# haowenz/chromap

Measured on AMD Instinct MI355X. Metric: M paired reads mapped/s (ATAC preset, GRCh38 index), higher is better.
Workload: dtype u64; 1 GPU; --preset atac, synthetic 2x50 bp pairs (fragments 30-600 bp, 1% substitutions), GRCh38-sized synthetic index (3.10e+09 bases, 24 sequences, k=17 w=7) resident per GPU, 4000000 pairs per GPU per step, 4 distinct batches per GPU resident in HBM taking turns (16 M distinct pairs per GPU); lanes=3, parallelism=single GPU

## Files before the change

chromap_amd/csrc/cm_api.hip:

```cpp
#include <hip/hip_runtime.h>
#include <math.h>
#include <stdio.h>
#include <stdlib.h>
#include <string.h>

#include <string>
#include <vector>

#include "../../include/chromap_amd.h"
#include "cm_barcode_translate.h"
#include "cm_ctx.h"
#include "cm_kernels.h"
#include "cm_classes.h"
#include "cm_summary.h"
#include "cm_coop.h"
#include <chrono>
#include <mutex>
#include "cm_mapq_tables.h"

static thread_local std::string g_last_error;

static bool cm_debug_pool() { static const bool on = getenv("CM_DEBUG_POOL") != nullptr; return on; }
static thread_local std::string t_last_error;
void cm_set_error(cmgpu_ctx *ctx, const std::string &msg) {
// ... 86 lines not shown
    c->opt.sam_group = (int)value;
  } else if (n == "verify_planes") {
    c->opt.planes = value ? 1 : 0;
  } else if (n == "speculative_sizes") {
    c->opt.spec = value ? 1 : 0;
    if (value < 0) { c->cls_seen = 0; memset(c->cls_age, 0, sizeof(c->cls_age)); }
  } else if (n == "debug_candidate_capacity") {
    if (value > 0 && cm_ensure_candidate_arrays(c, (uint64_t)value)) { cm_set_error(c, "out of device memory (candidates)"); return CMGPU_ENOMEM; }
    c->pred_m_ok = value > 0; c->m_cap = (uint64_t)value; c->pred_n = 0xffffffffu;
  } else if (n == "coop_profile") {
    if (value) { if (c->coop_prof.ensure(64 * 8)) return CMGPU_ENOMEM; CM_HIPCHECK(c, hipMemset(c->coop_prof.p, 0, 64 * 8)); } else c->coop_prof.release();
  } else if (n == "coop_run_table") {
    c->opt.coop_rb = (int)value;
  } else if (n == "coop") {
    c->opt.coop = (int)value;
  } else if (n == "s3b_short") {
    c->opt.s3b_short = value ? 1 : 0;
  } else if (n == "generic_kernels") {
    c->opt.generic_kernels = value ? 1 : 0;
  } else if (n == "item_limit") {
    c->opt.item_limit = value > 0 ? (uint64_t)value : 0xfffffff0ull;
  } else {
    cm_set_error(c, "unknown option " + n);
    return CMGPU_EINVAL;
  }
  return CMGPU_OK;
}

extern "C" int cmgpu_get_option(const cmgpu_ctx *c, const char *name, int64_t *value) {
  if (!c || !name || !value) return CMGPU_EINVAL;
  const std::string n(name);
  if (n == "probe_lookups_per_lane") *value = c->opt.probe_variant & 15;
  else if (n == "probe_pair_prefetch") *value = (c->opt.probe_variant & 16) ? 1 : 0;
  else if (n == "mm_chunks") *value = c->opt.mm_chunks;
  else if (n == "h2d_copy_blocks") *value = c->opt.h2d_kernel;
  else if (n == "d2h_copy_blocks") *value = c->opt.d2h_kernel;
  else if (n == "prep_kernel") *value = c->opt.prep_kernel;
  else if (n == "prep_tile_reads") *value = c->opt.prep_tile_reads;
  else if (n == "item_limit") *value = (int64_t)c->opt.item_limit;
  else if (n == "lanes") *value = c->opt.lanes;
  else if (n == "coop") *value = c->opt.coop;
  else if (n == "generic_kernels") *value = c->opt.generic_kernels;
  else if (n == "s3b_short") *value = c->opt.s3b_short;
  else if (n == "alloc_us") *value = (int64_t)(c->alloc_seconds * 1e6);
  else if (n == "alloc_draw_us") *value = (int64_t)(c->alloc_draw_seconds * 1e6);
  else if (n.rfind("coop_profile_", 0) == 0) {
    const int k = atoi(n.c_str() + 13);
    unsigned long long v = 0;
    if (k < 0 || k > 63 || !c->coop_prof.p || hipMemcpy(&v, (const unsigned long long *)c->coop_prof.p + k, 8, hipMemcpyDeviceToHost) != hipSuccess) return CMGPU_EINVAL;
    *value = (int64_t)v;
  }
  else if (n == "probe_table_buckets") *value = c->fmask ? (int64_t)c->fmask + 1 : (int64_t)c->bmask + 1;
  else return CMGPU_EINVAL;
  return CMGPU_OK;
}

extern "C" const char *cmgpu_last_error(const cmgpu_ctx *ctx) { return ctx ? ctx->err.c_str() : g_last_error.c_str(); }

// ... 621 lines not shown
#define CM_RC_AGAIN_ALL_CLASSES (-101)
#define CM_RC_AGAIN_EXACT_SIZES (-102)
struct RangeRun {
  cmgpu_ctx *c;
  uint32_t rlo, rhi, n, n2;
  bool allow_spec;
  uint64_t limit;
  hipStream_t s;
  CmDev d;
  uint32_t n_mm = 0;
  bool s3a_done = false;
  uint32_t n_heavy[CM_HV_LISTS] = {};
  unsigned long long hits_total = 0;
  uint32_t n_hits = 0;
  bool planes = false;
  bool spec = false;
  uint32_t n_m = 0;
  void bind() { cm_bind_dev(c, d, rlo, rhi); }
};
static int stage_begin(RangeRun &r) {
  cmgpu_ctx *c = r.c;
  c->n_ev = 0;
  c->use_perm = false;
  const int rc = ensure_pair_arrays(c, r.n);
  if (rc) return rc;
  CM_HIPCHECK(c, hipMemsetAsync(c->stats.p, 0, CM_ST_N * 8, r.s));
  memset(&r.d, 0, sizeof(r.d));
  cm_ensure_goff(c);
  cm_set_classes(c, r.d);
  r.bind();
// ... 19 lines not shown
static int mm_fill_and_probe(RangeRun &r, const MmChunks &k, uint32_t mm_cap, Fill fill) {
  cmgpu_ctx *c = r.c;
  const unsigned long long *marks = (const unsigned long long *)c->mm_marks.p;
  CM_HIPCHECK(c, hipMemsetAsync(r.d.stats + CM_ST_PROBE_STEPS, 0, 2 * 8, r.s));
  for (uint32_t ch = 0; ch < k.n_chunks; ++ch) {
    fill(ch);
    CM_HIPCHECK(c, hipEventRecord(c->chunk_ev[ch], r.s));
    CM_HIPCHECK(c, hipStreamWaitEvent(c->stream2, c->chunk_ev[ch], 0));
    cm_launch_k_probe_range(r.d, marks + ch, k.entries[ch], mm_cap, (uint2 *)c->partials.p + k.part_off[ch], c->stream2, c->opt.probe_variant);
  }
  CM_HIPCHECK(c, hipEventRecord(c->chunk_ev[CM_MM_CHUNKS], c->stream2));
  CM_HIPCHECK(c, hipStreamWaitEvent(r.s, c->chunk_ev[CM_MM_CHUNKS], 0));
  cm_launch_k_probe_reduce(c->partials.p, k.part_off[k.n_chunks], r.d.stats + CM_ST_PROBE_STEPS, r.s);
  return CMGPU_OK;
}
static int stage_minimizers_fused(RangeRun &r, bool flat) {
  cmgpu_ctx *c = r.c; CmDev &d = r.d; hipStream_t s = r.s;
  const uint32_t n = r.n, n2 = r.n2;
  int rc;
  uint64_t cap = (uint64_t)n2 * (c->max_read_len / 4 + 3);
  const uint64_t bound = (uint64_t)c->bases0 + c->bases1 + 1;
  if (cap > bound) cap = bound;
  const uint32_t ppb = flat ? 128u : cm_prep_mm_pairs_per_block(d, c->max_read_len);
  const uint64_t per_read_bound = c->max_read_len > (uint32_t)c->p.k ? c->max_read_len - (uint32_t)c->p.k + 1 : 1;
  MmChunks k;
  k.n_chunks = mm_chunk_count(r);
  for (int attempt = 0; attempt < 2; ++attempt) {
    if (cap > r.limit) return CM_RC_SPLIT;
    k.lo[0] = 0;
    uint32_t chunk_pairs = 0;
    for (uint32_t ch = 0; ch < k.n_chunks; ++ch) {
      uint64_t hi = (uint64_t)n * (ch + 1) / k.n_chunks;
      hi = ch + 1 == k.n_chunks ? n : hi / ppb * ppb;
      k.lo[ch + 1] = (uint32_t)hi;
// ... 3 lines not shown
      k.entries[ch] = me > cap ? cap : me;
    }
    mm_probe_grids(c, k);
    if (c->mm_hash.ensure((size_t)cap * 8 + 8) || c->mm_ps.ensure((size_t)cap * 4 + 4) || c->pr_val.ensure((size_t)cap * 8 + 8) ||
        (!flat && c->mm_stage.ensure(cm_prep_mm_stage_bytes(d, c->max_read_len, chunk_pairs) + 8)) ||
        c->pr_kind.ensure((size_t)cap + 4) || c->mm_cursor.ensure(8) || c->mm_marks.ensure((CM_MM_CHUNKS + 1) * 8) ||
        c->partials.ensure(((size_t)k.part_off[k.n_chunks] + 1) * 8 + cm_stats_partial_words(n) * 8)) {
      cm_set_error(c, "out of device memory (minimizers)"); return CMGPU_ENOMEM;
    }
    r.bind();
    CM_HIPCHECK(c, hipMemsetAsync(c->mm_cursor.p, 0, 8, s));
    CM_HIPCHECK(c, hipMemsetAsync(c->mm_marks.p, 0, 8, s));
    unsigned long long *cursor = (unsigned long long *)c->mm_cursor.p, *marks = (unsigned long long *)c->mm_marks.p;
    rc = mm_fill_and_probe(r, k, (uint32_t)cap, [&](uint32_t ch) {
      if (flat) cm_launch_k_prep_flat(d, k.lo[ch], k.lo[ch + 1], c->max_read_len, (uint32_t)c->opt.prep_tile_reads, (uint32_t)cap, cursor, s);
      else cm_launch_k_prep_mm(d, k.lo[ch], k.lo[ch + 1], c->max_read_len, (uint32_t)cap, cursor, s, c->mm_stage.p);
      cm_launch_k_copy_u64(cursor, marks + ch + 1, s);
    });
    if (rc) return rc;
    d.mm_cap = (uint32_t)cap;
    CM_HIPCHECK(c, hipMemsetAsync(c->hv_cnt.p, 0, 256, s));
    cm_launch_k_s3a_count(d, n2, s);
    d.mm_cap = 0;
    if ((rc = scan_with_total(c, d.hit_tot, d.hit_off, n2, &r.hits_total, false))) return rc;
    CM_HIPCHECK(c, hipMemcpyAsync(r.n_heavy, c->hv_cnt.p, sizeof(r.n_heavy), hipMemcpyDeviceToHost, s));
    r.s3a_done = true;
    unsigned long long hm[CM_MM_CHUNKS + 1];
    CM_HIPCHECK(c, hipMemcpyAsync(hm, marks, ((size_t)k.n_chunks + 1) * 8, hipMemcpyDeviceToHost, s));
    CM_HIPCHECK(c, cm_stream_sync(s));
    const unsigned long long tot = hm[k.n_chunks];
    bool grid_short = false;
// ... 24 lines not shown
  if (c->mm_marks.ensure((CM_MM_CHUNKS + 1) * 8)) { cm_set_error(c, "out of device memory (minimizers)"); return CMGPU_ENOMEM; }
  unsigned long long *marks = (unsigned long long *)c->mm_marks.p;
  unsigned long long hm[CM_MM_CHUNKS + 1];
  cm_launch_k_mm_marks(d.mm_off, k.lo, k.n_chunks + 1, marks, s);
  CM_HIPCHECK(c, hipMemcpyAsync(hm, marks, ((size_t)k.n_chunks + 1) * 8, hipMemcpyDeviceToHost, s));
  CM_HIPCHECK(c, cm_stream_sync(s));
  for (uint32_t ch = 0; ch < k.n_chunks; ++ch) k.entries[ch] = hm[ch + 1] - hm[ch];
  mm_probe_grids(c, k);
  if (c->partials.ensure(((size_t)k.part_off[k.n_chunks] + 1) * 8 + cm_stats_partial_words(r.n) * 8)) { cm_set_error(c, "out of device memory (partials)"); return CMGPU_ENOMEM; }
  if ((rc = mm_fill_and_probe(r, k, n_mm, [&](uint32_t ch) { cm_launch_k_mm_fill(d, k.lo[ch], k.lo[ch + 1], c->max_read_len, s); }))) return rc;
  mark(c, "s1b_s2_minimizers_probe");
  return CMGPU_OK;
}
static int stage_pack_reads(RangeRun &r) {
  cmgpu_ctx *c = r.c;
  r.planes = c->ref_pl_words != 0 && c->opt.planes;
  if (r.planes && c->read_planes.ensure((size_t)r.n2 * cm_read_pl_stride((c->max_read_len + 31) / 32) * 4 + 16)) r.planes = false;
  if (!r.planes) return CMGPU_OK;
  if (!c->stream_pack) {
    int prio_least = 0, prio_greatest = 0;
    (void)hipDeviceGetStreamPriorityRange(&prio_least, &prio_greatest);
    CM_HIPCHECK(c, hipStreamCreateWithPriority(&c->stream_pack, hipStreamNonBlocking, prio_greatest));
  }
  CM_HIPCHECK(c, hipEventRecord(c->chunk_ev[1], r.s));
  CM_HIPCHECK(c, hipStreamWaitEvent(c->stream_pack, c->chunk_ev[1], 0));
  r.d.read_pl = (uint32_t *)c->read_planes.p; r.d.read_pl_w = (c->max_read_len + 31) / 32;
  cm_launch_k_pack_reads(r.d, r.n2, c->stream_pack);
  CM_HIPCHECK(c, hipEventRecord(c->chunk_ev[0], c->stream_pack));
  return CMGPU_OK;
}
static int stage_s3_candidates(RangeRun &r) {
  cmgpu_ctx *c = r.c; CmDev &d = r.d; hipStream_t s = r.s;
// ... 70 lines not shown
  if (cm_debug_pool()) fprintf(stderr, "spec %d m_cap %llu m_total %llu\n", (int)r.spec, (unsigned long long)c->m_cap, m_total);
  r.bind();
  mark(c, "s4a_rescue_count");
  cm_launch_k_s4b_rescue_merge(d, n2, s, coop, c->max_read_len);
  cm_launch_k_s4b_rescue_list(d, n2, s, coop, c->max_read_len);
  mark(c, "s4b_rescue_merge");
  CM_HIPCHECK(c, hipMemsetAsync(c->srt_cnt.p, 0, 8, s));
  cm_launch_k_s4c_reduce(d, r.n, s, (uint32_t)c->opt.coop & (c->p.split ? ~8u : ~0u));
  if (c->use_perm) cm_launch_k_sort_lists(d, 0, s);
  mark(c, "s4c_pair_filter");
  return CMGPU_OK;
}
static int stage_s5_verify(RangeRun &r) {
  cmgpu_ctx *c = r.c; const CmDev &d = r.d; hipStream_t s = r.s;
  const bool coop = (c->opt.coop & 8) != 0 && !c->p.split;
  if (r.planes) CM_HIPCHECK(c, hipStreamWaitEvent(s, c->chunk_ev[0], 0));
  cm_launch_k_s5a_prepare(d, r.n2, s, coop);
  cm_scan_u32(d.nv, d.v_off, r.n2, (uint32_t *)c->scan_tmp.p, s);
  mark(c, "s5a_prepare");
  cm_launch_k_s5b_verify(d, r.n_m, r.n2, s);
  mark(c, "s5b_verify");
  CM_HIPCHECK(c, hipMemsetAsync(c->srt_cnt.p, 0, 8, s));
  cm_launch_k_s5c_finalize(d, r.n2, s, coop);
  if (c->use_perm) cm_launch_k_sort_lists(d, 1, s);
  mark(c, "s5c_accept");
  return CMGPU_OK;
}
static int stage_s6_records(RangeRun &r) {
  cmgpu_ctx *c = r.c; CmDev &d = r.d; hipStream_t s = r.s;
  const uint32_t n = r.n;
  const bool coop = (c->opt.coop & 16) != 0;
// ... 372 lines not shown
    t.force_mapq = c->p.split ? -1 : (f0[i] ? 0 : -1);
  }
  return CMGPU_OK;
}

extern "C" int cmgpu_debug_array(cmgpu_ctx *c, const char *name, uint32_t *out, uint64_t capacity, uint64_t *n_out) {
  if (!c || !name || !out) return CMGPU_EINVAL;
  CM_HIPCHECK(c, cm_enter(c));
  const std::string nm(name);
  if (nm == "hv_cnt") {
    if (n_out) *n_out = 64;
    if (capacity < 64 || !c->hv_cnt.p || c->hv_cnt.cap < 256) { cm_set_error(c, "debug array: buffer too small or array not resident"); return CMGPU_ECAPACITY; }
    CM_HIPCHECK(c, hipMemcpy(out, c->hv_cnt.p, 256, hipMemcpyDeviceToHost));
    return CMGPU_OK;
  }
  struct { const char *n; DevBuf *b; int per_pair; } tab[] = {
    {"rlen", &c->rlen, 0}, {"mm_cnt", &c->mm_cnt, 0}, {"hit_tot", &c->hit_tot, 0}, {"ncp", &c->ncp, 0}, {"ncn", &c->ncn, 0},
    {"resc_p", &c->resc_p, 0}, {"resc_n", &c->resc_n, 0}, {"mcp", &c->mcp, 0}, {"mcn", &c->mcn, 0}, {"fcp", &c->fcp, 0},
    {"fcn", &c->fcn, 0}, {"ndp", &c->ndp, 0}, {"ndn", &c->ndn, 0}, {"nv", &c->nv, 0}, {"pe_nbest", &c->pe_nbest, 1}};
  for (auto &t : tab)
    if (nm == t.n) {
      const uint64_t n = t.per_pair ? c->n_pairs : 2ull * c->n_pairs;
      if (n_out) *n_out = n;
      if (capacity < n || !t.b->p || t.b->cap < n * 4) { cm_set_error(c, "debug array: buffer too small or array not resident"); return CMGPU_ECAPACITY; }
      CM_HIPCHECK(c, hipMemcpy(out, t.b->p, n * 4, hipMemcpyDeviceToHost));
      return CMGPU_OK;
    }
  cm_set_error(c, "debug array: unknown name " + nm);
  return CMGPU_EINVAL;
}
// ... 528 lines not shown
```

chromap_amd/csrc/cm_ctx.h:

```cpp
#ifndef CM_CTX_H_
#define CM_CTX_H_
#include <hip/hip_runtime.h>

#include <string>
#include <thread>
#include <vector>

#include "../../include/chromap_amd.h"
#include "../../include/chromap_amd_debug.h"
#include "cm_types.h"

#define CM_MAX_EVENTS 32
#define CM_MAX_W_HOST 32

struct DevBuf {
  void *p = nullptr;
  size_t cap = 0;
  bool owned = true;
  int ensure(size_t bytes);
  void release();
};

struct CmTmpBuf : private DevBuf {
  using DevBuf::p;
// ... 85 lines not shown
  int sam_group = 8;
  int d2h_kernel = 0;
  int h2d_kernel = 0;
  int probe_variant = 1;
  int mm_chunks = CM_MM_CHUNKS;
  int prep_tile_reads = 32;
  int prep_kernel = 0;
  uint64_t item_limit = 0xfffffff0ull;
  int exchange_overlap = 0;
  int s3b_cap = 0;
  int lanes = 1;
  int heavy_mid = 0;
  int heavy_max[3] = {0, 0, 0};
  int heavy_last = 0;
  int spec = 1;
  int s3b_short = 1;
  int generic_kernels = 0;
  int coop_rb = 0;
  int coop = 0xff;
};

struct cmgpu_ctx {
  CmOptions opt;
  int device = 0;
  hipStream_t stream = nullptr;
  hipStream_t stream2 = nullptr;
  hipStream_t stream_pack = nullptr;
  hipEvent_t chunk_ev[CM_MM_CHUNKS + 1] = {};
  std::string err;
  cmgpu_params hp;
// ... 177 lines not shown
```

chromap_amd/csrc/cm_kernels.h:

```cpp
#ifndef CM_KERNELS_H_
#define CM_KERNELS_H_
#include <hip/hip_runtime.h>

#include "cm_types.h"

#define CM_SLAB_CAP 65535u
#define CM_SLAB_BLOCKS 128u
#define CM_DECL_LAUNCH(kname) void cm_launch_##kname(const CmDev &d, uint32_t n, hipStream_t s);
void cm_launch_k_prep_count(const CmDev &d, uint32_t n_pairs, uint32_t max_read_len, hipStream_t s);
void cm_launch_k_mm_fill(const CmDev &d, uint32_t pair_lo, uint32_t pair_hi, uint32_t max_read_len, hipStream_t s);
void cm_launch_k_mm_marks(const uint32_t *mm_off, const uint32_t *lo, uint32_t n_marks, unsigned long long *marks, hipStream_t s);
bool cm_prep_mm_supported(const CmDev &d, uint32_t max_read_len);
bool cm_prep_flat_supported(const CmDev &d, uint32_t max_read_len, uint32_t tile_reads);
void cm_launch_k_prep_flat(const CmDev &d, uint32_t pair_lo, uint32_t pair_hi, uint32_t max_read_len, uint32_t tile_reads, uint32_t mm_cap,
                           unsigned long long *cursor, hipStream_t s);
uint32_t cm_prep_mm_pairs_per_block(const CmDev &d, uint32_t max_read_len);
size_t cm_prep_mm_stage_bytes(const CmDev &d, uint32_t max_read_len, uint32_t pairs);
void cm_launch_k_prep_mm(const CmDev &d, uint32_t pair_lo, uint32_t pair_hi, uint32_t max_read_len, uint32_t mm_cap,
                         unsigned long long *cursor, hipStream_t s, void *gstage);
uint32_t cm_probe_range_blocks(uint64_t max_entries, int variant);
void cm_launch_k_probe_range(const CmDev &d, const unsigned long long *range, uint64_t max_entries, uint32_t cap, void *partials, hipStream_t s, int variant);
void cm_launch_k_probe_reduce(const void *partials, uint32_t blocks, unsigned long long *counters, hipStream_t s);
CM_DECL_LAUNCH(k_s3a_count)
void cm_launch_k_sort_lists(const CmDev &d, int mode, hipStream_t s);
uint32_t cm_s3b_lane_cap(uint32_t max_read_len);
void cm_s3b_heavy_classes(uint32_t *hv_max, uint32_t *hv_big);
void cm_granted_classes(CmDev &d);
void cm_launch_k_s3b_heavy(const CmDev &d, const uint32_t *n_cls, hipStream_t s, bool coop, uint32_t max_read_len);
void cm_launch_k_s3b_candidates(const CmDev &d, uint32_t n, uint32_t max_read_len, hipStream_t s);
void cm_launch_k_s4a_rescue_count(const CmDev &d, uint32_t n, hipStream_t s, bool coop);
void cm_launch_k_s4b_rescue_merge(const CmDev &d, uint32_t n, hipStream_t s, bool coop, uint32_t max_read_len);
uint32_t cm_rescue_seg_cap(uint32_t n_reads);
void cm_launch_k_s4a_rescue_list(const CmDev &d, uint32_t n_reads, hipStream_t s, bool coop);
void cm_launch_k_s4b_rescue_list(const CmDev &d, uint32_t n_reads, hipStream_t s, bool coop, uint32_t max_read_len);
// ... 30 lines not shown
```

chromap_amd/csrc/cm_kernels.hip:

```cpp
#include <hip/hip_runtime.h>
#include <stdio.h>
#include <string.h>
#include <cstring>
#include <atomic>
#include <map>
#include <mutex>
#include <type_traits>
#include <utility>
#include <rocprim/rocprim.hpp>

#include "cm_kernels.h"
#include "cm_stages.h"
#include "cm_classes.h"
#include "cm_coop.h"

#define CM_BLOCK 256

#define CM_ITEM_KERNEL(kname, fn, perm)                                      \
  __global__ __launch_bounds__(CM_BLOCK) void kname(CmDev d, uint32_t n) {   \
    if (d.abort && *d.abort) return;                                         \
    const uint32_t i = blockIdx.x * CM_BLOCK + threadIdx.x;                  \
    if (i < n) fn(d, d.perm ? d.perm[i] : i);                                \
  }

// ... 27 lines not shown
  const uint32_t t = threadIdx.x, lp = t < PB ? t : t - PB, pair = p0 + lp;
  const CmStaged s = cm_stage_pairs(d, p0, p1, pair, lds_half);
  if (t < PB && pair < p1) cm_s0_prep_ptr(d, pair, s.m0, s.m1);
  __syncthreads();
  if (pair < p1) cm_s1_count(d, 2 * pair + (t < PB ? 0 : 1), t < PB ? s.m0 : s.m1);
}

__global__ void k_mm_fill(CmDev d, uint32_t pair_lo, uint32_t n_pairs , uint32_t lds_half) {
  const uint32_t PB = blockDim.x >> 1;
  const uint32_t p0 = pair_lo + blockIdx.x * PB, p1 = p0 + PB < n_pairs ? p0 + PB : n_pairs;
  const uint32_t t = threadIdx.x, lp = t < PB ? t : t - PB, pair = p0 + lp;
  const CmStaged s = cm_stage_pairs(d, p0, p1, pair, lds_half);
  if (pair < p1) cm_s1_fill(d, 2 * pair + (t < PB ? 0 : 1), t < PB ? s.m0 : s.m1);
}

template <bool GSTAGE, bool E6>
__global__ void k_prep_mm(CmDev d, uint32_t pair_lo, uint32_t n_pairs , uint32_t lds_half, uint32_t stg,
                          uint32_t mm_cap, unsigned long long *cursor, uint64_t *gstage) {
  const uint32_t T = blockDim.x, PB = T >> 1;
  const uint32_t p0 = pair_lo + blockIdx.x * PB, p1 = p0 + PB < n_pairs ? p0 + PB : n_pairs;
  const uint32_t t = threadIdx.x, lp = t < PB ? t : t - PB, pair = p0 + lp;
  const CmStaged s = cm_stage_pairs(d, p0, p1, pair, lds_half);
  if (t < PB && pair < p1) cm_s0_prep_ptr(d, pair, s.m0, s.m1);
  __syncthreads();
  uint64_t *sh_e = GSTAGE ? gstage + (size_t)blockIdx.x * stg * T : reinterpret_cast<uint64_t *>(cm_lds + 2 * lds_half);
  uint32_t *sh_lo = reinterpret_cast<uint32_t *>(cm_lds + 2 * lds_half);
  uint16_t *sh_hi = reinterpret_cast<uint16_t *>(sh_lo + (size_t)stg * T);
  uint32_t *sh_w = reinterpret_cast<uint32_t *>(cm_lds + 2 * lds_half + (GSTAGE ? 0 : (size_t)stg * T * (E6 ? 6 : 8)));
  uint32_t *sh_off = sh_w + 16, *sh_cnt = sh_off + T + 1;
  const bool valid = pair < p1;
  const uint32_t r = 2 * pair + (t < PB ? 0 : 1);
  const uint8_t *seq = t < PB ? s.m0 : s.m1;
  const int k = d.p.k;
  const uint32_t hb = 2 * (uint32_t)k;
  uint32_t cnt = 0, len = 0;
  if (valid) {
    len = d.rlen[r];
    cnt = cm_minimizers_w7(seq, len, k, [&](uint32_t n, uint64_t h, uint32_t p) {
      const uint64_t v = h | ((uint64_t)p << hb);
      if (n < stg) { if (E6) { sh_lo[(size_t)n * T + t] = (uint32_t)v; sh_hi[(size_t)n * T + t] = (uint16_t)(v >> 32); } else sh_e[(size_t)n * T + t] = v; }
    });
  }
  const uint32_t lane = t & 63, wave = t >> 6;
  uint32_t incl = cnt;
#pragma unroll
  for (int dlt = 1; dlt < 64; dlt <<= 1) {
    const uint32_t v = __shfl_up(incl, dlt, 64);
    if (lane >= (uint32_t)dlt) incl += v;
  }
  if (lane == 63 || t == T - 1) sh_w[wave] = incl;
  __syncthreads();
  const uint32_t n_waves = (T + 63) >> 6;
  if (t == 0) {
    uint32_t tot = 0;
    for (uint32_t wv = 0; wv < n_waves; ++wv) { const uint32_t x = sh_w[wv]; sh_w[wv] = tot; tot += x; }
    const unsigned long long base = tot ? atomicAdd(cursor, (unsigned long long)tot) : 0ull;
// ... 1767 lines not shown
  return prep_mm_geometry(d, max_read_len, &t, &h, &g, &l);
}
uint32_t cm_prep_mm_pairs_per_block(const CmDev &d, uint32_t max_read_len) {
  uint32_t threads, half, stg;
  size_t lds;
  return prep_mm_geometry(d, max_read_len, &threads, &half, &stg, &lds) ? threads / 2 : 0;
}
size_t cm_prep_mm_stage_bytes(const CmDev &d, uint32_t max_read_len, uint32_t pairs) {
  uint32_t threads, half, stg;
  size_t lds;
  bool g = false;
  if (!prep_mm_geometry(d, max_read_len, &threads, &half, &stg, &lds, &g) || !g) return 0;
  const uint32_t pb = threads / 2;
  return (size_t)((pairs + pb - 1) / pb) * stg * threads * 8;
}
void cm_launch_k_prep_mm(const CmDev &d, uint32_t pair_lo, uint32_t pair_hi, uint32_t max_read_len, uint32_t mm_cap,
                         unsigned long long *cursor, hipStream_t s, void *gstage) {
  uint32_t threads, half, stg;
  size_t lds;
  bool g = false, e6 = false;
  if (pair_hi <= pair_lo || !prep_mm_geometry(d, max_read_len, &threads, &half, &stg, &lds, &g, &e6)) return;
  const uint32_t pb = threads / 2;
  if (g) hipLaunchKernelGGL((k_prep_mm<true, false>), dim3((pair_hi - pair_lo + pb - 1) / pb), dim3(threads), lds, s, d, pair_lo, pair_hi, half, stg, mm_cap, cursor, (uint64_t *)gstage);
  else if (e6) hipLaunchKernelGGL((k_prep_mm<false, true>), dim3((pair_hi - pair_lo + pb - 1) / pb), dim3(threads), lds, s, d, pair_lo, pair_hi, half, stg, mm_cap, cursor, (uint64_t *)nullptr);
  else hipLaunchKernelGGL((k_prep_mm<false, false>), dim3((pair_hi - pair_lo + pb - 1) / pb), dim3(threads), lds, s, d, pair_lo, pair_hi, half, stg, mm_cap, cursor, (uint64_t *)nullptr);
}
static inline int probe_variant_norm(int variant) {
  if (variant == 0) variant = CM_PROBE_U;
  const int u = variant & 15;
  return ((u == 2 || u == 4 || u == 8) ? u : 1) | (variant & 16);
}
uint32_t cm_probe_range_blocks(uint64_t max_entries, int variant) {
  const uint64_t per = (uint64_t)(probe_variant_norm(variant) & 15) * CM_BLOCK;
  return (uint32_t)((max_entries + per - 1) / per);
}
void cm_launch_k_probe_range(const CmDev &d, const unsigned long long *range, uint64_t max_entries, uint32_t cap, void *partials, hipStream_t s, int variant) {
  const uint32_t blocks = cm_probe_range_blocks(max_entries, variant);
  if (!blocks) return;
// ... 72 lines not shown
```

chromap_amd/csrc/cm_stages.h:

```cpp
#ifndef CM_STAGES_H_
#define CM_STAGES_H_

#include "cm_types.h"

struct CmModeAny {
  static constexpr bool kPe = false;
  static CM_HD bool split(const CmDev &d) { return d.p.split != 0; }
  static CM_HD bool single(const CmDev &d) { return d.p.single != 0; }
};
struct CmModePe {
  static constexpr bool kPe = true;
  static CM_HD bool split(const CmDev &) { return false; }
  static CM_HD bool single(const CmDev &) { return false; }
};

CM_HD uint32_t cm_c2u(uint8_t c) {
  const uint32_t u = c & 0xDFu;
  const uint32_t x = (u >> 1) & 3u;
  const uint32_t o = u - 0x41u;
  const bool acgt = o < 20u && ((0x80045u >> (o & 31u)) & 1u);
  return acgt ? x ^ (x >> 1) : 4u;
}
CM_HD uint8_t cm_negchar(uint8_t c) {
  const uint32_t v = 3u ^ cm_c2u(c);
// ... 400 lines not shown
    }
    const uint64_t r0 = d0 & seedmask;
    const uint64_t r1 = seed >= 32 ? d1 : (((d0 >> (2 * seed)) | (d1 << (64 - 2 * seed))) & seedmask);
    const bool ok = cnt <= 1;
    if (ok && r0 == 0) { fa = true; sa = s0; }
    if (ok && r1 == 0 && !fb) { fb = true; sb = s0; }
#pragma unroll
    for (int w = 0; w + 1 < W; ++w) b[w] = (b[w] >> 2) | (b[w + 1] << 62);
    b[W - 1] >>= 2;
  }
  *found = fa || fb;
  *s0_out = fa ? sa : sb;
  return true;
}

CM_HD void cm_s0_prep_ptr(const CmDev &d, uint32_t pair, const uint8_t *s1p, const uint8_t *s2p) {
  const uint32_t raw1 = d.ro0[pair + 1] - d.ro0[pair], raw2 = d.ro1[pair + 1] - d.ro1[pair];
  uint32_t len1 = raw1, len2 = raw2;
  bool ok = raw1 >= (uint32_t)d.p.min_read_len && (d.p.single || raw2 >= (uint32_t)d.p.min_read_len);
  if (d.bcb && !d.bc_ok[pair] && !d.p.bc_keep) ok = false;
  if (ok && d.p.trim && !d.p.single) {
    const uint8_t *s1 = s1p, *s2 = s2p;
    const bool swap = !(raw1 <= raw2);
    const uint8_t *rd1 = swap ? s2 : s1;
    const uint8_t *lng = swap ? s1 : s2;
    const uint32_t l1 = swap ? raw2 : raw1, l2 = swap ? raw1 : raw2;
    const int min_overlap = d.p.min_read_len;
    const int seed = min_overlap / 2;
    bool merged = false;
    bool fast = false, ffound = false;
    uint32_t fs0 = 0;
    if (seed >= 1 && seed <= 32 && 2 * seed <= min_overlap && l1 >= (uint32_t)min_overlap) {
      if (l2 <= 64) fast = cm_trim_fast<2>(rd1, l1, lng, l2, min_overlap, seed, &ffound, &fs0);
      else if (l2 <= 160) fast = cm_trim_fast<5>(rd1, l1, lng, l2, min_overlap, seed, &ffound, &fs0);
      else if (l2 <= 256) fast = cm_trim_fast<8>(rd1, l1, lng, l2, min_overlap, seed, &ffound, &fs0);
    }
    if (fast) {
      merged = true;
      if (ffound) {
        int overlap = (int)(l2 - fs0);
        int off2 = 0;
        if (overlap > (int)l1) { off2 = overlap - (int)l1; overlap = (int)l1; }
        const int t1 = swap ? overlap + off2 : overlap;
        const int t2 = swap ? overlap : overlap + off2;
        if (t1 < (int)raw1) len1 = (uint32_t)t1;
        if (t2 < (int)raw2) len2 = (uint32_t)t2;
      }
    }
// ... 101 lines not shown
        for (int j = 0; j < W; ++j)
          if (min_h == wh[j] && min_p != wp[j]) CM_EMIT(wh[j], wp[j]);
      }
    }
  }
  if (flush && min_h != ~0ull) CM_EMIT(min_h, min_p);
#undef CM_EMIT
  return n;
}

template <int W, class Emit>
CM_HD uint32_t cm_minimizers_window_e(const uint8_t *seq, uint32_t len, int k, Emit &&emit) {
  return cm_minimizers_core<W>(seq, 0, len, true, k, W, [&](uint32_t n, uint64_t h, uint32_t p) { emit(n, h, p); return true; });
}

template <class Emit>
CM_HD uint32_t cm_minimizers_w7_oddk_seq(const uint8_t *seq, uint32_t len, int k, Emit &&emit) {
  const uint64_t shift = 2 * (uint64_t)(k - 1);
  const uint64_t mask = (((uint64_t)1) << (2 * k)) - 1;
  uint64_t fw = 0, rv = 0;
  uint64_t H[7];
#pragma unroll
  for (int j = 0; j < 7; ++j) H[j] = ~0ull;
  uint32_t sb = 0, fl = 0, bad = 0, n = 0;
  for (uint32_t pos = 0; pos < len; ++pos) {
    uint32_t c = cm_c2u(seq[pos]);
    bad |= c >> 2;
    c &= 3;
    fw = ((fw << 2) | c) & mask;
    rv = (rv >> 2) | (((uint64_t)(3 ^ c)) << shift);
    if (pos + 1 < (uint32_t)k) continue;
    const uint64_t h0 = cm_hash64_k(fw, k, mask), h1 = cm_hash64_k(rv, k, mask);
    const uint32_t strand = h0 < h1 ? 0u : 1u;
    const uint64_t h = cm_hash64_k(strand ? h1 : h0, k, mask);
    if (fl & 1u) { emit(n, H[0], ((pos - 7) << 1) | (sb & 1u)); ++n; }
#pragma unroll
    for (int j = 0; j < 6; ++j) H[j] = H[j + 1];
    H[6] = h;
    sb = (sb >> 1) | (strand << 6);
    fl >>= 1;
    const uint32_t i = pos + 1 - (uint32_t)k;
// ... 20 lines not shown
  if (m_k < 7) {
    uint64_t v = ~0ull;
    int at = -1;
#pragma unroll
    for (int j = 0; j < 7; ++j)
      if (j >= 7 - (int)m_k && H[j] <= v) { v = H[j]; at = j; }
    if (at >= 0) { emit(n, v, ((len - 1 - (uint32_t)(6 - at)) << 1) | ((sb >> at) & 1u)); ++n; }
    return n;
  }
#pragma unroll
  for (int j = 0; j < 7; ++j)
    if ((fl >> j) & 1u) { emit(n, H[j], ((len - 1 - (uint32_t)(6 - j)) << 1) | ((sb >> j) & 1u)); ++n; }
  return n;
}

template <int HV, class Emit>
CM_HD uint32_t cm_minimizers_w7_oddk_blocks(const uint8_t *seq, uint32_t len, int k, Emit &&emit) {
  const uint64_t shift = 2 * (uint64_t)(k - 1);
  const uint64_t mask = (((uint64_t)1) << (2 * k)) - 1;
  uint64_t fw = 0, rv = 0;
  uint32_t bad = 0, n = 0;
  for (uint32_t pos = 0; pos + 1 < (uint32_t)k; ++pos) {
    uint32_t c = cm_c2u(seq[pos]);
    bad |= c >> 2;
    c &= 3;
    fw = ((fw << 2) | c) & mask;
    rv = (rv >> 2) | (((uint64_t)(3 ^ c)) << shift);
  }
  const uint32_t m = len - (uint32_t)k + 1, nblk = (m + 6) / 7;
  uint64_t ep[7], Sp[7], SM[7];
  uint32_t sbp = 0;
#pragma unroll
  for (int j = 0; j < 7; ++j) { ep[j] = 0; Sp[j] = 0; SM[j] = 0; }
  for (uint32_t b = 0; b <= nblk; ++b) {
    uint64_t e[7];
    uint32_t sb = 0;
#pragma unroll
    for (int j = 0; j < 7; ++j) {
      const uint32_t i = 7 * b + (uint32_t)j;
      e[j] = 0;
      if (i < m) {
        uint32_t c = cm_c2u(seq[i + (uint32_t)k - 1]);
        bad |= c >> 2;
        c &= 3;
        fw = ((fw << 2) | c) & mask;
        rv = (rv >> 2) | (((uint64_t)(3 ^ c)) << shift);
        const uint64_t h0 = cm_hash64_v<HV>(fw, mask), h1 = cm_hash64_v<HV>(rv, mask);
        const uint32_t strand = h0 < h1 ? 0u : 1u;
        e[j] = cm_hash64_v<HV>(strand ? h1 : h0, mask);
        sb |= strand << j;
      }
    }
    if (b == 0) {
      uint64_t v = e[0];
#pragma unroll
      for (int j = 1; j < 6; ++j) v = e[j] < v ? e[j] : v;
      if (e[6] == v) {
// ... 23 lines not shown
    }
    SM[6] = Mw[6];
    Sp[6] = e[6];
#pragma unroll
    for (int j = 5; j >= 0; --j) {
      SM[j] = Mw[j] > SM[j + 1] ? Mw[j] : SM[j + 1];
      Sp[j] = e[j] < Sp[j + 1] ? e[j] : Sp[j + 1];
    }
#pragma unroll
    for (int j = 0; j < 7; ++j) ep[j] = e[j];
    sbp = sb;
  }
  if (bad) return ~0u;
  return n;
}
template <class Emit>
CM_HD uint32_t cm_minimizers_w7_oddk(const uint8_t *seq, uint32_t len, int k, Emit &&emit) {
  if (len < (uint32_t)k + 6) return cm_minimizers_w7_oddk_seq(seq, len, k, emit);
  if (2 * k == 34) return cm_minimizers_w7_oddk_blocks<0>(seq, len, k, emit);
  if (2 * k > 32 && 2 * k <= 52) return cm_minimizers_w7_oddk_blocks<1>(seq, len, k, emit);
  return cm_minimizers_w7_oddk_blocks<2>(seq, len, k, emit);
}

CM_HD uint32_t cm_mmf_pack4(uint32_t w, uint32_t *bad4) {
  const uint32_t x = (w >> 1) & 0x03030303u;
  const uint32_t code = x ^ ((x >> 1) & 0x01010101u);
  const uint32_t b0 = code & 0x01010101u, b1 = (code >> 1) & 0x01010101u;
  const uint32_t canon = 0x41414141u + 2u * b0 + 6u * b1 + 11u * (b0 & b1);
  const uint32_t diff = (w & 0xDFDFDFDFu) ^ canon;
  const uint32_t nz = ((diff & 0x7F7F7F7Fu) + 0x7F7F7F7Fu) | diff;
  const uint32_t m = (nz >> 7) & 0x01010101u;
  *bad4 = (m | (m >> 7) | (m >> 14) | (m >> 21)) & 0xFu;
  uint32_t t = (code | (code >> 6)) & 0x000F000Fu;
  t = (t | (t >> 12)) & 0xFFu;
  return t;
}
// ... 33 lines not shown
  for (uint32_t i = 0; i < m; ++i) {
    const uint32_t j0 = i >= 6 ? i - 6 : 0, j1 = i + 7 <= m ? i : m - 7;
    uint64_t x = 0;
    for (uint32_t j = j0; j <= j1; ++j) x = Mbuf[j] > x ? Mbuf[j] : x;
    flag[i] = x == h[i] ? 1 : 0;
  }
  return true;
}

template <class Emit>
CM_HD uint32_t cm_minimizers_w7(const uint8_t *seq, uint32_t len, int k, Emit &&emit) {
  if (k & 1) {
    const uint32_t n = cm_minimizers_w7_oddk(seq, len, k, emit);
    if (n != ~0u) return n;
  }
  return cm_minimizers_window_e<7>(seq, len, k, emit);
}

template <int W>
CM_HD uint32_t cm_minimizers_window(const uint8_t *seq, uint32_t len, int k, uint64_t *oh, uint32_t *op, uint32_t cap) {
  auto put = [&](uint32_t n, uint64_t h, uint32_t p) { if (oh && n < cap) { oh[n] = h; op[n] = p; } };
  if (W == 7) return cm_minimizers_w7(seq, len, k, put);
  return cm_minimizers_window_e<W>(seq, len, k, put);
}

CM_HD uint32_t cm_minimizers_ring(const uint8_t *seq, uint32_t len, int k, int w, uint64_t *oh, uint32_t *op, uint32_t cap) {
  return cm_minimizers_core<0>(seq, 0, len, true, k, w, [&](uint32_t n, uint64_t h, uint32_t p) {
    if (oh && n < cap) { oh[n] = h; op[n] = p; }
    return true;
  });
// ... 1172 lines not shown
    Q x = {o[i], i + 1 < 6 * W ? o[i + 1] : 0u, i + 2 < 6 * W ? o[i + 2] : 0u, i + 3 < 6 * W ? o[i + 3] : 0u};
    *reinterpret_cast<Q *>(dst + i) = x;
  }
}
CM_HD void cm_pack_read_planes(const CmDev &d, uint32_t r) {
  switch (d.read_pl_w) {
    case 1: cm_pack_read_planes_w<1>(d, r); break;
    case 2: cm_pack_read_planes_w<2>(d, r); break;
    case 3: cm_pack_read_planes_w<3>(d, r); break;
    case 4: cm_pack_read_planes_w<4>(d, r); break;
    case 5: cm_pack_read_planes_w<5>(d, r); break;
    case 6: cm_pack_read_planes_w<6>(d, r); break;
    case 7: cm_pack_read_planes_w<7>(d, r); break;
    case 8: cm_pack_read_planes_w<8>(d, r); break;
    default: cm_pack_read_planes_any(d, r);
  }
}

CM_HD uint64_t cm_load8(const uint8_t *p) {
  const uintptr_t a = reinterpret_cast<uintptr_t>(p);
  const uint32_t sh = (uint32_t)(a & 7) * 8;
  const uint64_t *ap = reinterpret_cast<const uint64_t *>(a & ~(uintptr_t)7);
  const uint64_t lo = ap[0];
  if (sh == 0) return lo;
  return (lo >> sh) | (ap[1] << (64 - sh));
}
CM_HD uint64_t cm_swar_eq(uint64_t v, uint64_t k) {
  const uint64_t z = v ^ (k * 0x0101010101010101ull);
  const uint64_t m = ~(((z & 0x7F7F7F7F7F7F7F7Full) + 0x7F7F7F7F7F7F7F7Full) | z) & 0x8080808080808080ull;
  return (m >> 7) * 0xFFull;
// ... 1296 lines not shown
```

Baseline: 570.0 M pairs/s.

## Pack read bit-planes once in prep kernel and reuse for trim, minimizers, verify

For reads up to 64 bp, the minimizer prep kernel now packs each read into 2-bit planes in registers. It shares the mate's planes through shared memory so adapter trimming can run on popcounted plane XORs, feeds odd-k minimizer extraction from the planes instead of bytes, and writes the read-plane array used by verification directly. This removes the separate pack-reads pass, its extra stream and event wait, and repeated byte decoding. In exchange the prep kernel gains register pressure and an occupancy hint, plus an extra block barrier.

```diff
diff --git a/chromap_amd/csrc/cm_api.hip b/chromap_amd/csrc/cm_api.hip
--- a/chromap_amd/csrc/cm_api.hip
+++ b/chromap_amd/csrc/cm_api.hip
@@ -124,6 +124,8 @@
     c->opt.coop_rb = (int)value;
   } else if (n == "coop") {
     c->opt.coop = (int)value;
+  } else if (n == "pack_once") {
+    c->opt.pack_once = value ? 1 : 0;
   } else if (n == "s3b_short") {
     c->opt.s3b_short = value ? 1 : 0;
   } else if (n == "generic_kernels") {
@@ -152,6 +154,7 @@
   else if (n == "coop") *value = c->opt.coop;
   else if (n == "generic_kernels") *value = c->opt.generic_kernels;
   else if (n == "s3b_short") *value = c->opt.s3b_short;
+  else if (n == "pack_once") *value = c->opt.pack_once;
   else if (n == "alloc_us") *value = (int64_t)(c->alloc_seconds * 1e6);
   else if (n == "alloc_draw_us") *value = (int64_t)(c->alloc_draw_seconds * 1e6);
   else if (n.rfind("coop_profile_", 0) == 0) {
@@ -803,6 +806,7 @@
   unsigned long long hits_total = 0;
   uint32_t n_hits = 0;
   bool planes = false;
+  bool planes_in_prep = false;
   bool spec = false;
   uint32_t n_m = 0;
   void bind() { cm_bind_dev(c, d, rlo, rhi); }
@@ -852,10 +856,17 @@
   cm_launch_k_probe_reduce(c->partials.p, k.part_off[k.n_chunks], r.d.stats + CM_ST_PROBE_STEPS, r.s);
   return CMGPU_OK;
 }
+static bool range_wants_planes(const cmgpu_ctx *c) { return c->ref_pl_words != 0 && c->opt.planes; }
+static size_t read_planes_bytes(const cmgpu_ctx *c, uint32_t n2) { return (size_t)n2 * cm_read_pl_stride((c->max_read_len + 31) / 32) * 4 + 16; }
 static int stage_minimizers_fused(RangeRun &r, bool flat) {
   cmgpu_ctx *c = r.c; CmDev &d = r.d; hipStream_t s = r.s;
   const uint32_t n = r.n, n2 = r.n2;
   int rc;
+  const bool pl = !flat && c->opt.pack_once && cm_prep_mm_planes_supported(d, c->max_read_len);
+  if (pl && range_wants_planes(c) && !c->read_planes.ensure(read_planes_bytes(c, n2))) {
+    d.read_pl = (uint32_t *)c->read_planes.p; d.read_pl_w = (c->max_read_len + 31) / 32;
+    r.planes_in_prep = true;
+  }
   uint64_t cap = (uint64_t)n2 * (c->max_read_len / 4 + 3);
   const uint64_t bound = (uint64_t)c->bases0 + c->bases1 + 1;
   if (cap > bound) cap = bound;
@@ -889,7 +900,7 @@
     unsigned long long *cursor = (unsigned long long *)c->mm_cursor.p, *marks = (unsigned long long *)c->mm_marks.p;
     rc = mm_fill_and_probe(r, k, (uint32_t)cap, [&](uint32_t ch) {
       if (flat) cm_launch_k_prep_flat(d, k.lo[ch], k.lo[ch + 1], c->max_read_len, (uint32_t)c->opt.prep_tile_reads, (uint32_t)cap, cursor, s);
-      else cm_launch_k_prep_mm(d, k.lo[ch], k.lo[ch + 1], c->max_read_len, (uint32_t)cap, cursor, s, c->mm_stage.p);
+      else cm_launch_k_prep_mm(d, k.lo[ch], k.lo[ch + 1], c->max_read_len, (uint32_t)cap, cursor, s, c->mm_stage.p, pl);
       cm_launch_k_copy_u64(cursor, marks + ch + 1, s);
     });
     if (rc) return rc;
@@ -944,8 +955,9 @@
 }
 static int stage_pack_reads(RangeRun &r) {
   cmgpu_ctx *c = r.c;
-  r.planes = c->ref_pl_words != 0 && c->opt.planes;
-  if (r.planes && c->read_planes.ensure((size_t)r.n2 * cm_read_pl_stride((c->max_read_len + 31) / 32) * 4 + 16)) r.planes = false;
+  r.planes = range_wants_planes(c);
+  if (r.planes_in_prep) return CMGPU_OK;
+  if (r.planes && c->read_planes.ensure(read_planes_bytes(c, r.n2))) r.planes = false;
   if (!r.planes) return CMGPU_OK;
   if (!c->stream_pack) {
     int prio_least = 0, prio_greatest = 0;
@@ -1046,7 +1058,7 @@
 static int stage_s5_verify(RangeRun &r) {
   cmgpu_ctx *c = r.c; const CmDev &d = r.d; hipStream_t s = r.s;
   const bool coop = (c->opt.coop & 8) != 0 && !c->p.split;
-  if (r.planes) CM_HIPCHECK(c, hipStreamWaitEvent(s, c->chunk_ev[0], 0));
+  if (r.planes && !r.planes_in_prep) CM_HIPCHECK(c, hipStreamWaitEvent(s, c->chunk_ev[0], 0));
   cm_launch_k_s5a_prepare(d, r.n2, s, coop);
   cm_scan_u32(d.nv, d.v_off, r.n2, (uint32_t *)c->scan_tmp.p, s);
   mark(c, "s5a_prepare");
@@ -1449,6 +1461,14 @@
     CM_HIPCHECK(c, hipMemcpy(out, c->hv_cnt.p, 256, hipMemcpyDeviceToHost));
     return CMGPU_OK;
   }
+  if (nm == "read_pl") {
+    const uint64_t n = 2ull * c->n_pairs * cm_read_pl_stride((c->max_read_len + 31) / 32);
+    if (n_out) *n_out = n;
+    if (c->last_range_lo != 0 || c->last_range_hi != c->n_pairs) { cm_set_error(c, "the batch was mapped in sub-batches"); return CMGPU_EINVAL; }
+    if (capacity < n || !c->read_planes.p || c->read_planes.cap < n * 4) { cm_set_error(c, "debug array: buffer too small or array not resident"); return CMGPU_ECAPACITY; }
+    CM_HIPCHECK(c, hipMemcpy(out, c->read_planes.p, n * 4, hipMemcpyDeviceToHost));
+    return CMGPU_OK;
+  }
   struct { const char *n; DevBuf *b; int per_pair; } tab[] = {
     {"rlen", &c->rlen, 0}, {"mm_cnt", &c->mm_cnt, 0}, {"hit_tot", &c->hit_tot, 0}, {"ncp", &c->ncp, 0}, {"ncn", &c->ncn, 0},
     {"resc_p", &c->resc_p, 0}, {"resc_n", &c->resc_n, 0}, {"mcp", &c->mcp, 0}, {"mcn", &c->mcn, 0}, {"fcp", &c->fcp, 0},
diff --git a/chromap_amd/csrc/cm_ctx.h b/chromap_amd/csrc/cm_ctx.h
--- a/chromap_amd/csrc/cm_ctx.h
+++ b/chromap_amd/csrc/cm_ctx.h
@@ -123,6 +123,7 @@
   int heavy_max[3] = {0, 0, 0};
   int heavy_last = 0;
   int spec = 1;
+  int pack_once = 1;
   int s3b_short = 1;
   int generic_kernels = 0;
   int coop_rb = 0;
diff --git a/chromap_amd/csrc/cm_kernels.h b/chromap_amd/csrc/cm_kernels.h
--- a/chromap_amd/csrc/cm_kernels.h
+++ b/chromap_amd/csrc/cm_kernels.h
@@ -16,8 +16,9 @@
                            unsigned long long *cursor, hipStream_t s);
 uint32_t cm_prep_mm_pairs_per_block(const CmDev &d, uint32_t max_read_len);
 size_t cm_prep_mm_stage_bytes(const CmDev &d, uint32_t max_read_len, uint32_t pairs);
+bool cm_prep_mm_planes_supported(const CmDev &d, uint32_t max_read_len);
 void cm_launch_k_prep_mm(const CmDev &d, uint32_t pair_lo, uint32_t pair_hi, uint32_t max_read_len, uint32_t mm_cap,
-                         unsigned long long *cursor, hipStream_t s, void *gstage);
+                         unsigned long long *cursor, hipStream_t s, void *gstage, bool planes = false);
 uint32_t cm_probe_range_blocks(uint64_t max_entries, int variant);
 void cm_launch_k_probe_range(const CmDev &d, const unsigned long long *range, uint64_t max_entries, uint32_t cap, void *partials, hipStream_t s, int variant);
 void cm_launch_k_probe_reduce(const void *partials, uint32_t blocks, unsigned long long *counters, hipStream_t s);
diff --git a/chromap_amd/csrc/cm_kernels.hip b/chromap_amd/csrc/cm_kernels.hip
--- a/chromap_amd/csrc/cm_kernels.hip
+++ b/chromap_amd/csrc/cm_kernels.hip
@@ -65,14 +65,32 @@
   if (pair < p1) cm_s1_fill(d, 2 * pair + (t < PB ? 0 : 1), t < PB ? s.m0 : s.m1);
 }
 
-template <bool GSTAGE, bool E6>
-__global__ void k_prep_mm(CmDev d, uint32_t pair_lo, uint32_t n_pairs , uint32_t lds_half, uint32_t stg,
+template <bool GSTAGE, bool E6, bool PL = false>
+__global__ __attribute__((amdgpu_waves_per_eu(PL ? 6 : 1))) void k_prep_mm(CmDev d, uint32_t pair_lo, uint32_t n_pairs , uint32_t lds_half, uint32_t stg,
                           uint32_t mm_cap, unsigned long long *cursor, uint64_t *gstage) {
+  static_assert(!(PL && GSTAGE), "the planes route stages its emissions in shared memory");
   const uint32_t T = blockDim.x, PB = T >> 1;
   const uint32_t p0 = pair_lo + blockIdx.x * PB, p1 = p0 + PB < n_pairs ? p0 + PB : n_pairs;
   const uint32_t t = threadIdx.x, lp = t < PB ? t : t - PB, pair = p0 + lp;
   const CmStaged s = cm_stage_pairs(d, p0, p1, pair, lds_half);
-  if (t < PB && pair < p1) cm_s0_prep_ptr(d, pair, s.m0, s.m1);
+  uint64_t pl0 = 0, pl1 = 0, pln = 0;
+  if (PL) {
+    uint64_t *xp = reinterpret_cast<uint64_t *>(cm_lds + 2 * lds_half);
+    uint32_t *xu = reinterpret_cast<uint32_t *>(xp + 2 * (size_t)T);
+    if (pair < p1) {
+      const uint32_t raw = t < PB ? d.ro0[pair + 1] - d.ro0[pair] : d.ro1[pair + 1] - d.ro1[pair];
+      uint64_t plu;
+      cm_read_planes64(t < PB ? s.m0 : s.m1, raw, &pl0, &pl1, &pln, &plu);
+      xp[t] = pl0; xp[T + t] = pl1; xu[t] = (plu & cm_mask64(raw)) == 0 ? 1u : 0u;
+    }
+    __syncthreads();
+    if (t < PB && pair < p1) {
+      CmPairPlanes pp;
+      pp.p0[0] = pl0; pp.p1[0] = pl1; pp.upper[0] = xu[t] != 0;
+      pp.p0[1] = xp[t + PB]; pp.p1[1] = xp[T + t + PB]; pp.upper[1] = xu[t + PB] != 0;
+      cm_s0_prep_ptr(d, pair, s.m0, s.m1, &pp);
+    }
+  } else if (t < PB && pair < p1) cm_s0_prep_ptr(d, pair, s.m0, s.m1);
   __syncthreads();
   uint64_t *sh_e = GSTAGE ? gstage + (size_t)blockIdx.x * stg * T : reinterpret_cast<uint64_t *>(cm_lds + 2 * lds_half);
   uint32_t *sh_lo = reinterpret_cast<uint32_t *>(cm_lds + 2 * lds_half);
@@ -87,10 +105,14 @@
   uint32_t cnt = 0, len = 0;
   if (valid) {
     len = d.rlen[r];
-    cnt = cm_minimizers_w7(seq, len, k, [&](uint32_t n, uint64_t h, uint32_t p) {
+    auto put = [&](uint32_t n, uint64_t h, uint32_t p) {
       const uint64_t v = h | ((uint64_t)p << hb);
       if (n < stg) { if (E6) { sh_lo[(size_t)n * T + t] = (uint32_t)v; sh_hi[(size_t)n * T + t] = (uint16_t)(v >> 32); } else sh_e[(size_t)n * T + t] = v; }
-    });
+    };
+    if (PL) {
+      if (d.read_pl) cm_finish_read_planes(d, r, pl0, pl1, pln, len);
+      cnt = cm_minimizers_w7_planes(pl0, pl1, (pln & cm_mask64(len)) != 0, seq, len, k, put);
+    } else cnt = cm_minimizers_w7(seq, len, k, put);
   }
   const uint32_t lane = t & 63, wave = t >> 6;
   uint32_t incl = cnt;
@@ -1888,14 +1910,24 @@
   const uint32_t pb = threads / 2;
   return (size_t)((pairs + pb - 1) / pb) * stg * threads * 8;
 }
+bool cm_prep_mm_planes_supported(const CmDev &d, uint32_t max_read_len) {
+  uint32_t threads, half, stg;
+  size_t lds;
+  bool g = false, e6 = false;
+  if (max_read_len > 64 || !prep_mm_geometry(d, max_read_len, &threads, &half, &stg, &lds, &g, &e6) || g) return false;
+  return (size_t)stg * (e6 ? 6 : 8) >= 20;
+}
 void cm_launch_k_prep_mm(const CmDev &d, uint32_t pair_lo, uint32_t pair_hi, uint32_t max_read_len, uint32_t mm_cap,
-                         unsigned long long *cursor, hipStream_t s, void *gstage) {
+                         unsigned long long *cursor, hipStream_t s, void *gstage, bool planes) {
   uint32_t threads, half, stg;
   size_t lds;
   bool g = false, e6 = false;
   if (pair_hi <= pair_lo || !prep_mm_geometry(d, max_read_len, &threads, &half, &stg, &lds, &g, &e6)) return;
   const uint32_t pb = threads / 2;
-  if (g) hipLaunchKernelGGL((k_prep_mm<true, false>), dim3((pair_hi - pair_lo + pb - 1) / pb), dim3(threads), lds, s, d, pair_lo, pair_hi, half, stg, mm_cap, cursor, (uint64_t *)gstage);
+  if (planes && cm_prep_mm_planes_supported(d, max_read_len)) {
+    if (e6) hipLaunchKernelGGL((k_prep_mm<false, true, true>), dim3((pair_hi - pair_lo + pb - 1) / pb), dim3(threads), lds, s, d, pair_lo, pair_hi, half, stg, mm_cap, cursor, (uint64_t *)nullptr);
+    else hipLaunchKernelGGL((k_prep_mm<false, false, true>), dim3((pair_hi - pair_lo + pb - 1) / pb), dim3(threads), lds, s, d, pair_lo, pair_hi, half, stg, mm_cap, cursor, (uint64_t *)nullptr);
+  } else if (g) hipLaunchKernelGGL((k_prep_mm<true, false>), dim3((pair_hi - pair_lo + pb - 1) / pb), dim3(threads), lds, s, d, pair_lo, pair_hi, half, stg, mm_cap, cursor, (uint64_t *)gstage);
   else if (e6) hipLaunchKernelGGL((k_prep_mm<false, true>), dim3((pair_hi - pair_lo + pb - 1) / pb), dim3(threads), lds, s, d, pair_lo, pair_hi, half, stg, mm_cap, cursor, (uint64_t *)nullptr);
   else hipLaunchKernelGGL((k_prep_mm<false, false>), dim3((pair_hi - pair_lo + pb - 1) / pb), dim3(threads), lds, s, d, pair_lo, pair_hi, half, stg, mm_cap, cursor, (uint64_t *)nullptr);
 }
diff --git a/chromap_amd/csrc/cm_stages.h b/chromap_amd/csrc/cm_stages.h
--- a/chromap_amd/csrc/cm_stages.h
+++ b/chromap_amd/csrc/cm_stages.h
@@ -438,7 +438,31 @@
   return true;
 }
 
-CM_HD void cm_s0_prep_ptr(const CmDev &d, uint32_t pair, const uint8_t *s1p, const uint8_t *s2p) {
+CM_HD uint32_t cm_brev32(uint32_t v);
+CM_HD uint64_t cm_brev64(uint64_t v) { return ((uint64_t)cm_brev32((uint32_t)v) << 32) | cm_brev32((uint32_t)(v >> 32)); }
+CM_HD uint64_t cm_mask64(uint32_t n) { return n >= 64u ? ~0ull : ((1ull << n) - 1ull); }
+CM_HD void cm_trim_planes64(uint64_t a0, uint64_t a1, uint32_t l1, uint64_t b0, uint64_t b1, uint32_t l2, int min_overlap, int seed,
+                            bool *found, uint32_t *s0_out) {
+  const uint32_t down = 64u - l2;
+  uint64_t B0 = ~(cm_brev64(b0) >> down), B1 = ~(cm_brev64(b1) >> down);
+  const uint64_t seedmask = cm_mask64((uint32_t)seed);
+  bool fa = false, fb = false;
+  uint32_t sa = 0, sb = 0;
+  const uint32_t last = l2 - (uint32_t)min_overlap;
+  for (uint32_t s0 = 0; s0 <= last && !fa; ++s0) {
+    const uint32_t n = l1 < l2 - s0 ? l1 : l2 - s0;
+    const uint64_t D = ((a0 ^ B0) | (a1 ^ B1)) & cm_mask64(n);
+    const bool ok = __builtin_popcountll(D) <= 1;
+    if (ok && (D & seedmask) == 0) { fa = true; sa = s0; }
+    if (ok && ((D >> seed) & seedmask) == 0 && !fb) { fb = true; sb = s0; }
+    B0 >>= 1; B1 >>= 1;
+  }
+  *found = fa || fb;
+  *s0_out = fa ? sa : sb;
+}
+struct CmPairPlanes { uint64_t p0[2], p1[2]; bool upper[2]; };
+
+CM_HD void cm_s0_prep_ptr(const CmDev &d, uint32_t pair, const uint8_t *s1p, const uint8_t *s2p, const CmPairPlanes *pp = nullptr) {
   const uint32_t raw1 = d.ro0[pair + 1] - d.ro0[pair], raw2 = d.ro1[pair + 1] - d.ro1[pair];
   uint32_t len1 = raw1, len2 = raw2;
   bool ok = raw1 >= (uint32_t)d.p.min_read_len && (d.p.single || raw2 >= (uint32_t)d.p.min_read_len);
@@ -455,7 +479,11 @@
     bool fast = false, ffound = false;
     uint32_t fs0 = 0;
     if (seed >= 1 && seed <= 32 && 2 * seed <= min_overlap && l1 >= (uint32_t)min_overlap) {
-      if (l2 <= 64) fast = cm_trim_fast<2>(rd1, l1, lng, l2, min_overlap, seed, &ffound, &fs0);
+      if (pp && l2 <= 64) {
+        const int ia = swap ? 1 : 0, ib = swap ? 0 : 1;
+        fast = pp->upper[0] && pp->upper[1];
+        if (fast) cm_trim_planes64(pp->p0[ia], pp->p1[ia], l1, pp->p0[ib], pp->p1[ib], l2, min_overlap, seed, &ffound, &fs0);
+      } else if (l2 <= 64) fast = cm_trim_fast<2>(rd1, l1, lng, l2, min_overlap, seed, &ffound, &fs0);
       else if (l2 <= 160) fast = cm_trim_fast<5>(rd1, l1, lng, l2, min_overlap, seed, &ffound, &fs0);
       else if (l2 <= 256) fast = cm_trim_fast<8>(rd1, l1, lng, l2, min_overlap, seed, &ffound, &fs0);
     }
@@ -587,8 +615,16 @@
   return cm_minimizers_core<W>(seq, 0, len, true, k, W, [&](uint32_t n, uint64_t h, uint32_t p) { emit(n, h, p); return true; });
 }
 
-template <class Emit>
-CM_HD uint32_t cm_minimizers_w7_oddk_seq(const uint8_t *seq, uint32_t len, int k, Emit &&emit) {
+struct CmSrcBytes {
+  const uint8_t *seq;
+  CM_HD uint32_t operator()(uint32_t i) const { return cm_c2u(seq[i]); }
+};
+struct CmSrcPlanes {
+  uint64_t p0, p1;
+  CM_HD uint32_t operator()(uint32_t i) const { return ((uint32_t)(p0 >> i) & 1u) | (((uint32_t)(p1 >> i) & 1u) << 1); }
+};
+template <class Src, class Emit>
+CM_HD uint32_t cm_minimizers_w7_oddk_seq_src(const Src &src, uint32_t len, int k, Emit &&emit) {
   const uint64_t shift = 2 * (uint64_t)(k - 1);
   const uint64_t mask = (((uint64_t)1) << (2 * k)) - 1;
   uint64_t fw = 0, rv = 0;
@@ -597,7 +633,7 @@
   for (int j = 0; j < 7; ++j) H[j] = ~0ull;
   uint32_t sb = 0, fl = 0, bad = 0, n = 0;
   for (uint32_t pos = 0; pos < len; ++pos) {
-    uint32_t c = cm_c2u(seq[pos]);
+    uint32_t c = src(pos);
     bad |= c >> 2;
     c &= 3;
     fw = ((fw << 2) | c) & mask;
@@ -648,14 +684,14 @@
   return n;
 }
 
-template <int HV, class Emit>
-CM_HD uint32_t cm_minimizers_w7_oddk_blocks(const uint8_t *seq, uint32_t len, int k, Emit &&emit) {
+template <int HV, class Src, class Emit>
+CM_HD uint32_t cm_minimizers_w7_oddk_blocks_src(const Src &src, uint32_t len, int k, Emit &&emit) {
   const uint64_t shift = 2 * (uint64_t)(k - 1);
   const uint64_t mask = (((uint64_t)1) << (2 * k)) - 1;
   uint64_t fw = 0, rv = 0;
   uint32_t bad = 0, n = 0;
   for (uint32_t pos = 0; pos + 1 < (uint32_t)k; ++pos) {
-    uint32_t c = cm_c2u(seq[pos]);
+    uint32_t c = src(pos);
     bad |= c >> 2;
     c &= 3;
     fw = ((fw << 2) | c) & mask;
@@ -674,7 +710,7 @@
       const uint32_t i = 7 * b + (uint32_t)j;
       e[j] = 0;
       if (i < m) {
-        uint32_t c = cm_c2u(seq[i + (uint32_t)k - 1]);
+        uint32_t c = src(i + (uint32_t)k - 1);
         bad |= c >> 2;
         c &= 3;
         fw = ((fw << 2) | c) & mask;
@@ -728,12 +764,24 @@
   if (bad) return ~0u;
   return n;
 }
+template <class Src, class Emit>
+CM_HD uint32_t cm_minimizers_w7_oddk_src(const Src &src, uint32_t len, int k, Emit &&emit) {
+  if (len < (uint32_t)k + 6) return cm_minimizers_w7_oddk_seq_src(src, len, k, emit);
+  if (2 * k == 34) return cm_minimizers_w7_oddk_blocks_src<0>(src, len, k, emit);
+  if (2 * k > 32 && 2 * k <= 52) return cm_minimizers_w7_oddk_blocks_src<1>(src, len, k, emit);
+  return cm_minimizers_w7_oddk_blocks_src<2>(src, len, k, emit);
+}
+template <class Emit>
+CM_HD uint32_t cm_minimizers_w7_oddk_seq(const uint8_t *seq, uint32_t len, int k, Emit &&emit) {
+  return cm_minimizers_w7_oddk_seq_src(CmSrcBytes{seq}, len, k, emit);
+}
+template <int HV, class Emit>
+CM_HD uint32_t cm_minimizers_w7_oddk_blocks(const uint8_t *seq, uint32_t len, int k, Emit &&emit) {
+  return cm_minimizers_w7_oddk_blocks_src<HV>(CmSrcBytes{seq}, len, k, emit);
+}
 template <class Emit>
 CM_HD uint32_t cm_minimizers_w7_oddk(const uint8_t *seq, uint32_t len, int k, Emit &&emit) {
-  if (len < (uint32_t)k + 6) return cm_minimizers_w7_oddk_seq(seq, len, k, emit);
-  if (2 * k == 34) return cm_minimizers_w7_oddk_blocks<0>(seq, len, k, emit);
-  if (2 * k > 32 && 2 * k <= 52) return cm_minimizers_w7_oddk_blocks<1>(seq, len, k, emit);
-  return cm_minimizers_w7_oddk_blocks<2>(seq, len, k, emit);
+  return cm_minimizers_w7_oddk_src(CmSrcBytes{seq}, len, k, emit);
 }
 
 CM_HD uint32_t cm_mmf_pack4(uint32_t w, uint32_t *bad4) {
@@ -797,6 +845,12 @@
     const uint32_t n = cm_minimizers_w7_oddk(seq, len, k, emit);
     if (n != ~0u) return n;
   }
+  return cm_minimizers_window_e<7>(seq, len, k, emit);
+}
+
+template <class Emit>
+CM_HD uint32_t cm_minimizers_w7_planes(uint64_t p0, uint64_t p1, bool bad, const uint8_t *seq, uint32_t len, int k, Emit &&emit) {
+  if ((k & 1) && !bad) return cm_minimizers_w7_oddk_src(CmSrcPlanes{p0, p1}, len, k, emit);
   return cm_minimizers_window_e<7>(seq, len, k, emit);
 }
 
@@ -1999,6 +2053,43 @@
     case 7: cm_pack_read_planes_w<7>(d, r); break;
     case 8: cm_pack_read_planes_w<8>(d, r); break;
     default: cm_pack_read_planes_any(d, r);
+  }
+}
+
+CM_HD void cm_read_planes64(const uint8_t *read, uint32_t len, uint64_t *p0, uint64_t *p1, uint64_t *pn, uint64_t *pu) {
+  const uintptr_t ra = reinterpret_cast<uintptr_t>(read);
+  const uint32_t sh8 = (uint32_t)(ra & 7) * 8;
+  const uint64_t *ap = reinterpret_cast<const uint64_t *>(ra & ~(uintptr_t)7);
+  uint64_t wv[9];
+#pragma unroll
+  for (int q = 0; q <= 8; ++q) wv[q] = (uint32_t)q * 8u < (sh8 >> 3) + len ? ap[q] : 0ull;
+  uint64_t q0 = 0, q1 = 0, qn = 0, qu = 0;
+#pragma unroll
+  for (int g = 0; g < 8; ++g) {
+    if (8u * (uint32_t)g >= len) break;
+    const uint64_t v = sh8 ? (wv[g] >> sh8) | (wv[g + 1] << (64u - sh8)) : wv[g];
+    const uint32_t a = (uint32_t)v, b = (uint32_t)(v >> 32);
+    uint32_t b0, b1, bn;
+    cm_pack8_planes(a, b, &b0, &b1, &bn);
+    const uint32_t lc = cm_fold8(((a >> 5) & 0x01010101u) | (((b >> 5) & 0x01010101u) << 4));
+    q0 |= (uint64_t)b0 << (8 * g); q1 |= (uint64_t)b1 << (8 * g); qn |= (uint64_t)bn << (8 * g); qu |= (uint64_t)(bn | lc) << (8 * g);
+  }
+  *p0 = q0; *p1 = q1; *pn = qn; *pu = qu;
+}
+CM_HD void cm_finish_read_planes(const CmDev &d, uint32_t r, uint64_t p0, uint64_t p1, uint64_t pn, uint32_t L) {
+  if (L == 0) return;
+  const uint64_t fn = pn | ~cm_mask64(L), f0 = p0 & ~fn, f1 = p1 & ~fn;
+  const uint32_t down = 64u - (L < 64u ? L : 64u);
+  const uint64_t r0 = ~(cm_brev64(f0) >> down), r1 = ~(cm_brev64(f1) >> down), rn = cm_brev64(fn) >> down;
+  uint32_t *dst = cm_read_pl_of(d, r);
+  struct alignas(16) Q { uint32_t a, b, c, e; };
+  if (d.read_pl_w == 1) {
+    *reinterpret_cast<Q *>(dst) = Q{(uint32_t)f0, (uint32_t)f1, (uint32_t)fn, (uint32_t)r0};
+    *reinterpret_cast<Q *>(dst + 4) = Q{(uint32_t)r1, (uint32_t)rn, 0u, 0u};
+  } else {
+    *reinterpret_cast<Q *>(dst) = Q{(uint32_t)f0, (uint32_t)(f0 >> 32), (uint32_t)f1, (uint32_t)(f1 >> 32)};
+    *reinterpret_cast<Q *>(dst + 4) = Q{(uint32_t)fn, (uint32_t)(fn >> 32), (uint32_t)r0, (uint32_t)(r0 >> 32)};
+    *reinterpret_cast<Q *>(dst + 8) = Q{(uint32_t)r1, (uint32_t)(r1 >> 32), (uint32_t)rn, (uint32_t)(rn >> 32)};
   }
 }
 
```

New measurement: 588.9 M pairs/s (median of 6 runs). 1.03x the previous value.
